# IBM/spark-s3-shuffle

Hardware: AMD Instinct MI355X
Metric: shuffle_block_compress_checksum_throughput (higher is better)
Workload: dtype u8; 1 GPU; terasort-10g-200p-lz4; direction=compress, codec=lz4, checksum=adler32, partitions_per_map_task=200, map_task_bytes=134217700, map_tasks_per_gpu=8, task_threads_per_gpu=4, map_tasks_per_library_call=2, inputs=resident in HBM

## Files before the change

### include/s3shuffle_codec.h

```cpp
#ifndef S3SHUFFLE_CODEC_H
#define S3SHUFFLE_CODEC_H

#include <stdint.h>

#ifdef __cplusplus
extern "C" {
#endif

#define S3S_ABI_VERSION 11

enum { S3S_CODEC_NONE = 0, S3S_CODEC_LZ4 = 1, S3S_CODEC_SNAPPY = 2,
       S3S_CODEC_LZF = 4,
       S3S_CODEC_ZSTD = 3  };
enum { S3S_CHECKSUM_NONE = 0, S3S_CHECKSUM_ADLER32 = 1, S3S_CHECKSUM_CRC32 = 2,
       S3S_CHECKSUM_CRC32C = 3  };

enum {
  S3S_OK = 0,
  S3S_E_INVALID = -1,
  S3S_E_CAPACITY = -2,
  S3S_E_BAD_FRAME = -3,
  S3S_E_CHECKSUM = -4,
  S3S_E_HIP = -5,
  S3S_E_UNSUPPORTED = -6,
  S3S_E_NOMEM = -7,
  S3S_STATUS_NOT_RUN = -100
};

enum {
  S3S_OPT_LZ4_BLOCK_SIZE = 1,
  S3S_OPT_SNAPPY_BLOCK_SIZE = 2,
  S3S_OPT_PROFILE = 3,
  S3S_OPT_LZ4_VARIANT = 4,
  S3S_OPT_LZ4_VARIANT_USED = 7,
  S3S_OPT_SNAPPY_VARIANT = 6,
  S3S_OPT_LZ4_DECODE_VARIANT = 5,
  S3S_OPT_LZ4_BLOCK_SIZE_LARGE = 8,
  S3S_OPT_ZSTD_COMPRESS = 9,
  S3S_OPT_LZF_COMPRESS = 10,
  S3S_OPT_IO_ENCRYPTION_KEY_BITS = 11
};

enum {
  S3S_STAGE_TOTAL = 0,
  S3S_STAGE_CODEC = 1,
  S3S_STAGE_ASSEMBLE = 2,
  S3S_STAGE_CHECKSUM = 3,
  S3S_STAGE_DISCOVER = 4,
  S3S_STAGE_HASH = 5,
  S3S_STAGE_COUNT = 6
};

typedef struct s3s_ctx s3s_ctx;

const char* s3s_version(void);
int s3s_abi_version(void);
int s3s_device_count(void);
s3s_ctx* s3s_create(int device_ordinal, int64_t scratch_bytes);
void s3s_destroy(s3s_ctx* ctx);
const char* s3s_last_error(const s3s_ctx* ctx);
int s3s_set_option(s3s_ctx* ctx, int key, int64_t value);
int64_t s3s_get_option(const s3s_ctx* ctx, int key);
int s3s_set_io_encryption(s3s_ctx* ctx, const uint8_t* key, int32_t key_bytes);
int s3s_set_stream_ivs(s3s_ctx* ctx, const uint8_t* ivs, int64_t n_ivs);
void* s3s_stream(const s3s_ctx* ctx);
double s3s_stage_ms(const s3s_ctx* ctx, int stage);

int64_t s3s_max_compressed_size(const s3s_ctx* ctx, int codec, const int64_t* src_offsets,
                                int32_t num_partitions);

int s3s_compress_map_output(s3s_ctx* ctx, int codec, int checksum_algo, const uint8_t* src,
                            const int64_t* src_offsets, int32_t num_partitions, uint8_t* dst,
                            int64_t dst_capacity, int64_t* out_index, int64_t* out_checksums,
// ... 105 lines not shown
```

### spark-s3-shuffle_amd/csrc/codec_api.hip

```cpp
#include "s3s_ctx.h"
#include <atomic>

using namespace s3s;

namespace {
inline void dbg_sync(s3s_ctx* ctx, const char* what) {
  static const bool on = getenv("S3S_DEBUG_SYNC") != nullptr;
  if (!on) return;
  const hipError_t e = hipStreamSynchronize(ctx->stream);
  fprintf(stderr, "[s3s] %s: %s\n", what, hipGetErrorString(e));
}
}

extern "C" {

const char* s3s_version(void) { return "s3shuffle-codec-mi355x 0.1.0 (gfx950)"; }
int s3s_abi_version(void) { return S3S_ABI_VERSION; }

int s3s_device_count(void) {
  int n = 0;
  if (hipGetDeviceCount(&n) != hipSuccess) return 0;
  return n;
}

s3s_ctx* s3s_create(int device_ordinal, int64_t scratch_bytes) {
  int n = 0;
  hipError_t e = hipGetDeviceCount(&n);
  if (e != hipSuccess || n <= 0) {
    fail(nullptr, S3S_E_HIP, "no HIP device available (%s); this library has no CPU fallback",
         e != hipSuccess ? hipGetErrorString(e) : "device count 0");
    return nullptr;
  }
  if (device_ordinal < 0 || device_ordinal >= n) {
    fail(nullptr, S3S_E_INVALID, "device ordinal %d out of range [0,%d)", device_ordinal, n);
    return nullptr;
  }
  s3s_ctx* ctx = new s3s_ctx();
  ctx->device = device_ordinal;
  auto bail = [&](const char* what, hipError_t err) -> s3s_ctx* {
    fail(nullptr, S3S_E_HIP, "%s failed: %s", what, hipGetErrorString(err));
    delete ctx;
    return nullptr;
  };
  if ((e = hipSetDevice(device_ordinal)) != hipSuccess) return bail("hipSetDevice", e);
  {
    int cus = 0;
    if (hipDeviceGetAttribute(&cus, hipDeviceAttributeMultiprocessorCount, device_ordinal) == hipSuccess && cus > 0) ctx->cu_count = cus;
  }
  if ((e = hipStreamCreateWithFlags(&ctx->stream, hipStreamNonBlocking)) != hipSuccess)
    return bail("hipStreamCreate", e);
  for (auto& ev : ctx->ev)
    if ((e = hipEventCreate(&ev)) != hipSuccess) return bail("hipEventCreate", e);
  if ((e = hipEventCreate(&ctx->ev_hash)) != hipSuccess) return bail("hipEventCreate", e);
  for (auto& ev : ctx->ev_auto)
    if ((e = hipEventCreate(&ev)) != hipSuccess) return bail("hipEventCreate", e);
  const size_t tb = checksum_tables_bytes();
  std::vector<uint8_t> host_tabs(tb);
  checksum_tables_build(host_tabs.data());
  if (ensure(ctx, B_TABLES, tb) != S3S_OK ||
      hipMemcpy(ctx->buf[B_TABLES].p, host_tabs.data(), tb, hipMemcpyHostToDevice) != hipSuccess) {
    fail(nullptr, S3S_E_HIP, "table upload failed: %s", ctx->err);
    s3s_destroy(ctx);
    return nullptr;
  }
  if (scratch_bytes > 0) (void)ensure(ctx, B_SLOTS, (size_t)scratch_bytes);
  return ctx;
}

void s3s_destroy(s3s_ctx* ctx) {
  if (!ctx) return;
  hipSetDevice(ctx->device);
  if (ctx->stream) hipStreamSynchronize(ctx->stream);
  if (ctx->hb_shared) {
    for (int i = 0; i < 2; i++) {
      if (ctx->hb_ev_in[i]) hipEventSynchronize(ctx->hb_ev_in[i]);
      if (ctx->hb_ev_out[i]) hipEventSynchronize(ctx->hb_ev_out[i]);
    }
  } else {
    if (ctx->hb_in) hipStreamSynchronize(ctx->hb_in);
    if (ctx->hb_out) hipStreamSynchronize(ctx->hb_out);
  }
  for (auto& b : ctx->buf)
    if (b.p) hipFree(b.p);
  if (ctx->h_stage) hipHostFree(ctx->h_stage);
  for (auto& ev : ctx->ev)
    if (ev) hipEventDestroy(ev);
  if (ctx->ev_hash) hipEventDestroy(ctx->ev_hash);
  for (auto& ev : ctx->ev_auto)
    if (ev) hipEventDestroy(ev);
  for (auto& ev : ctx->ev_up)
    if (ev) hipEventDestroy(ev);
  if (ctx->copy_stream) hipStreamDestroy(ctx->copy_stream);
  for (int i = 0; i < 2; i++) {
    if (ctx->hb_ev_in[i]) hipEventDestroy(ctx->hb_ev_in[i]);
    if (ctx->hb_ev_out[i]) hipEventDestroy(ctx->hb_ev_out[i]);
  }
  if (ctx->hb_in && !ctx->hb_shared) hipStreamDestroy(ctx->hb_in);
  if (ctx->hb_out && !ctx->hb_shared) hipStreamDestroy(ctx->hb_out);
  if (ctx->stream) hipStreamDestroy(ctx->stream);
  wipe(&ctx->enc_keys, sizeof ctx->enc_keys);
  delete ctx;
}

void* s3s_host_alloc(int64_t bytes) {
  if (bytes <= 0) return nullptr;
  void* p = nullptr;
  if (hipHostMalloc(&p, (size_t)bytes, hipHostMallocPortable) != hipSuccess) return nullptr;
  return p;
}

void s3s_host_free(void* p) {
  if (p) (void)hipHostFree(p);
}

const char* s3s_last_error(const s3s_ctx* ctx) { return ctx ? ctx->err : g_create_error; }

int s3s_set_option(s3s_ctx* ctx, int key, int64_t value) {
  if (!ctx) return S3S_E_INVALID;
  switch (key) {
    case S3S_OPT_LZ4_BLOCK_SIZE:
      if (value < 64) return fail(ctx, S3S_E_INVALID, "lz4 blockSize must be >= 64, got %lld", (long long)value);
      if (value > kLz4MaxBlock)
        return fail(ctx, S3S_E_UNSUPPORTED, "lz4 blockSize %lld > %d not supported", (long long)value, kLz4MaxBlock);
      ctx->lz4_block = value;
      return S3S_OK;
    case S3S_OPT_LZ4_BLOCK_SIZE_LARGE:
      if (value < 64) return fail(ctx, S3S_E_INVALID, "lz4 blockSize must be >= 64, got %lld", (long long)value);
      if (value > kBatchMaxBlock)
        return fail(ctx, S3S_E_UNSUPPORTED, "lz4 blockSize %lld > %d not supported", (long long)value, kBatchMaxBlock);
      ctx->lz4_block = value;
      return S3S_OK;
    case S3S_OPT_SNAPPY_BLOCK_SIZE:
      if (value <= 0) return fail(ctx, S3S_E_INVALID, "snappy blockSize must be > 0");
      if (value > kBatchMaxBlock)
        return fail(ctx, S3S_E_UNSUPPORTED, "snappy blockSize %lld > %d not supported", (long long)value, kBatchMaxBlock);
      ctx->snappy_block = value;
      return S3S_OK;
    case S3S_OPT_PROFILE:
      ctx->profile = value != 0;
      return S3S_OK;
    case S3S_OPT_ZSTD_COMPRESS:
      if (value != 0 && value != 1) return fail(ctx, S3S_E_INVALID, "zstd compress must be 0 or 1");
      ctx->zstd_compress = (int)value;
      return S3S_OK;
    case S3S_OPT_LZF_COMPRESS:
      if (value != 0 && value != 1) return fail(ctx, S3S_E_INVALID, "lzf compress must be 0 or 1");
      ctx->lzf_compress = (int)value;
      return S3S_OK;
    case S3S_OPT_LZ4_DECODE_VARIANT:
      if (value != 3 && value != 4) return fail(ctx, S3S_E_INVALID, "decode variant must be 3 (ring decoder) or 4 (batch decoder)");
      ctx->lz4_decode_variant = (int)value;
      return S3S_OK;
    case S3S_OPT_SNAPPY_VARIANT:
      if (value < 0 || value > 1) return fail(ctx, S3S_E_INVALID, "snappy variant must be 0..1");
      ctx->snappy_variant = (int)value;
      return S3S_OK;
    case S3S_OPT_LZ4_VARIANT:
      if (value != 1 && value != 9 && value != 10) return fail(ctx, S3S_E_INVALID, "lz4 variant must be 1 (general batch), 10 (exact windows) or 9 (auto)");
      ctx->lz4_variant = (int)value;
      ctx->auto_samples[0] = ctx->auto_samples[1] = 0;
      ctx->auto_tick = 0;
      return S3S_OK;
    case S3S_OPT_IO_ENCRYPTION_KEY_BITS:
      return fail(ctx, S3S_E_INVALID, "option %d is read-only (s3s_set_io_encryption switches the layer)", key);
  }
  return fail(ctx, S3S_E_INVALID, "unknown option %d", key);
}

int64_t s3s_get_option(const s3s_ctx* ctx, int key) {
  if (!ctx) return S3S_E_INVALID;
  switch (key) {
    case S3S_OPT_LZ4_BLOCK_SIZE:
    case S3S_OPT_LZ4_BLOCK_SIZE_LARGE: return ctx->lz4_block;
    case S3S_OPT_SNAPPY_BLOCK_SIZE: return ctx->snappy_block;
    case S3S_OPT_PROFILE: return ctx->profile;
    case S3S_OPT_LZ4_VARIANT: return ctx->lz4_variant;
    case S3S_OPT_LZ4_VARIANT_USED: return ctx->lz4_variant_used;
    case S3S_OPT_LZ4_DECODE_VARIANT: return ctx->lz4_decode_variant;
    case S3S_OPT_SNAPPY_VARIANT: return ctx->snappy_variant;
    case S3S_OPT_ZSTD_COMPRESS: return ctx->zstd_compress;
    case S3S_OPT_LZF_COMPRESS: return ctx->lzf_compress;
    case S3S_OPT_IO_ENCRYPTION_KEY_BITS: return ctx->enc_key_bits;
  }
  return S3S_E_INVALID;
}

int s3s_set_io_encryption(s3s_ctx* ctx, const uint8_t* key, int32_t key_bytes) {
  if (!ctx) return S3S_E_INVALID;
  ctx->err[0] = 0;
  if (!key || key_bytes == 0) {
    wipe(&ctx->enc_keys, sizeof ctx->enc_keys);
    ctx->enc_rounds = ctx->enc_key_bits = 0;
    ctx->enc_epoch++;
    return S3S_OK;
  }
  if (key_bytes != 16 && key_bytes != 24 && key_bytes != 32)
    return fail(ctx, S3S_E_INVALID, "IO encryption key must be 16, 24 or 32 bytes, got %d", (int)key_bytes);
  AesKeys fresh = {};
  const int rounds = aes_expand_key(key, key_bytes, &fresh);
  ctx->enc_keys = fresh;
  wipe(&fresh, sizeof fresh);
  ctx->enc_rounds = rounds;
  ctx->enc_key_bits = 8 * key_bytes;
  ctx->enc_epoch++;
  return S3S_OK;
}

int s3s_set_stream_ivs(s3s_ctx* ctx, const uint8_t* ivs, int64_t n_ivs) {
  if (!ctx) return S3S_E_INVALID;
  ctx->err[0] = 0;
  ctx->ivs.clear();
  ctx->ivs_set = false;
  if (n_ivs < 0 || (n_ivs > 0 && !ivs)) return fail(ctx, S3S_E_INVALID, "null IV array or negative count");
  if (n_ivs > 0x7fffffffll) return fail(ctx, S3S_E_INVALID, "more IVs than a call has partitions");
  ctx->ivs.assign(ivs, ivs + 16 * (size_t)n_ivs);
// ... 392 lines not shown
      k.status = s3s_compress_map_output_device(ctx, codec, checksum_algo, k.d_src, k.src_offsets, k.num_partitions,
                                                k.d_dst, k.dst_capacity, k.out_index, k.out_checksums, &k.out_total);
      if (k.status != S3S_OK && worst == S3S_OK) worst = k.status;
    }
    return verdict.finish(worst);
  }
  HIP_TRY(ctx, hipSetDevice(ctx->device));
  const int64_t bs = effective_block(ctx, codec);
  const int level = codec == S3S_CODEC_LZ4 ? lz4_level(bs) : 0;
  int64_t n_items64 = 0, n_chunks64 = 0, n_parts64 = 0;
  for (int32_t t = 0; t < n_tasks; t++) {
    const s3s_map_task& k = tasks[t];
    if (k.num_partitions < 0 || !k.src_offsets || !k.out_index || k.dst_capacity < 0)
      return fail(ctx, S3S_E_INVALID, "task %d: null offsets/index, negative partition count or capacity", t);
    if (checksum_algo != S3S_CHECKSUM_NONE && !k.out_checksums)
      return fail(ctx, S3S_E_INVALID, "task %d: out_checksums is null but a checksum algorithm is selected", t);
    for (int32_t p = 0; p < k.num_partitions; p++) {
      const int64_t u = k.src_offsets[p + 1] - k.src_offsets[p];
      if (u < 0) return fail(ctx, S3S_E_INVALID, "task %d: offsets not monotonic at %d", t, p);
      if (u > 0 && codec == S3S_CODEC_SNAPPY) {
        snappy_segment_counts(bs, u, &n_items64, &n_chunks64);
      } else if (u > 0) {
        const int64_t ch = (u + bs - 1) / bs;
        n_chunks64 += ch;
        n_items64 += ch + (codec != S3S_CODEC_LZF);
      }
    }
    const int64_t tu = k.num_partitions > 0 ? k.src_offsets[k.num_partitions] - k.src_offsets[0] : 0;
    if ((tu > 0 && !k.d_src) || (!k.d_dst && k.dst_capacity > 0)) return fail(ctx, S3S_E_INVALID, "task %d: null data pointer", t);
    n_parts64 += k.num_partitions;
  }
  if (n_items64 > 0x7fffff00ll) return fail(ctx, S3S_E_UNSUPPORTED, "too many codec blocks in one call");
  const int32_t n_items = (int32_t)n_items64, n_chunks = (int32_t)n_chunks64;
  const size_t np1 = (size_t)n_parts64 + (size_t)n_tasks;
  const size_t items_bytes = sizeof(Item) * (size_t)n_items;
  auto al = [](size_t x) { return (x + 15) & ~size_t(15); };
  const size_t o_items = 0, o_pf = al(o_items + items_bytes), o_seg = al(o_pf + 4 * np1), o_idx = al(o_seg + 4 * np1),
               o_sums = al(o_idx + 8 * np1), o_status = al(o_sums + 8 * ((size_t)n_parts64 + 1)),
               o_tails = al(o_status + 4 * (size_t)n_tasks + 16), stage_total = o_tails + sizeof(TaskTail) * (size_t)n_tasks + 16;
  int rc;
  if ((rc = ensure_stage(ctx, stage_total))) return rc;
  uint8_t* hs = static_cast<uint8_t*>(ctx->h_stage);
  Item* h_items = reinterpret_cast<Item*>(hs + o_items);
  int32_t* h_pf = reinterpret_cast<int32_t*>(hs + o_pf);
  int32_t* h_seg = reinterpret_cast<int32_t*>(hs + o_seg);
  int64_t* h_idx = reinterpret_cast<int64_t*>(hs + o_idx);
  int64_t* h_sums = reinterpret_cast<int64_t*>(hs + o_sums);
  int32_t* h_status = reinterpret_cast<int32_t*>(hs + o_status);
  TaskTail* h_tails = reinterpret_cast<TaskTail*>(hs + o_tails);
  std::vector<int32_t> first_item((size_t)n_tasks + 1), first_part((size_t)n_tasks + 1), first_seg((size_t)n_tasks + 1);
  const uint8_t* base = tasks[0].d_src;
  {
    int32_t it = 0, ch = 0, pp = 0, seg = 0;
    for (int32_t t = 0; t < n_tasks; t++) {
      const s3s_map_task& k = tasks[t];
      first_item[(size_t)t] = it;
      first_part[(size_t)t] = pp;
      first_seg[(size_t)t] = seg;
      const int64_t delta = k.d_src ? (int64_t)(k.d_src - base) : 0;
      int32_t* pf = h_pf + pp + t;
      int32_t* sg = h_seg + pp + t;
      int32_t seg_t = 0;
      for (int32_t p = 0; p < k.num_partitions; p++) {
        pf[p] = it - first_item[(size_t)t];
        sg[p] = seg_t;
        const int64_t u = k.src_offsets[p + 1] - k.src_offsets[p];
        seg_t += worst_segs(max_partition_size(codec, bs, u));
        if (u <= 0) continue;
        if (codec == S3S_CODEC_SNAPPY) h_items[it++] = Item{0, 0, kItemSnappyHeader, -1, p};
        if (codec == S3S_CODEC_ZSTD) h_items[it++] = Item{u, 0, kItemZstdHeader, -1, p};
        for (int64_t pos = 0; pos < u; pos += bs) {
          const int32_t len = (int32_t)((u - pos) < bs ? (u - pos) : bs);
          if (codec == S3S_CODEC_SNAPPY) {
            snappy_plan_chunk(h_items, it, ch, delta + k.src_offsets[p] + pos, len, p);
            continue;
          }
          if (codec == S3S_CODEC_ZSTD) {
            h_items[it++] = Item{delta + k.src_offsets[p] + pos, len, kItemZstdBlock | ((pos + len == u) << 8), ch++, p};
            continue;
          }
          if (codec == S3S_CODEC_LZF) {
            h_items[it++] = Item{delta + k.src_offsets[p] + pos, len, kItemLzfChunk, ch++, p};
            continue;
          }
          h_items[it++] = Item{delta + k.src_offsets[p] + pos, len, lz4_chunk_kind(len) | (level << 8), ch++, p};
        }
        if (codec == S3S_CODEC_LZ4) h_items[it++] = Item{0, 0, kItemLz4End | (level << 8), -1, p};
      }
      pf[k.num_partitions] = it - first_item[(size_t)t];
      sg[k.num_partitions] = seg_t;
      seg += seg_t;
      pp += k.num_partitions;
    }
    first_item[(size_t)n_tasks] = it;
    first_part[(size_t)n_tasks] = pp;
    first_seg[(size_t)n_tasks] = seg;
  }
  const int32_t total_segs = first_seg[(size_t)n_tasks];
  const int64_t slot_stride = codec == S3S_CODEC_SNAPPY ? snappy_slot_stride(bs) : codec_slot_stride(codec, bs);
  if ((rc = ensure(ctx, B_ITEMS, items_bytes + 16))) return rc;
  if ((rc = ensure(ctx, B_PART_FIRST, 4 * np1))) return rc;
  if ((rc = ensure(ctx, B_SEG_START, 4 * np1))) return rc;
  if ((rc = ensure(ctx, B_INDEX, 8 * np1))) return rc;
  if ((rc = ensure(ctx, B_SUMS, 8 * ((size_t)n_parts64 + 1)))) return rc;
  if ((rc = ensure(ctx, B_STATUS, 4 * (size_t)n_tasks + 16))) return rc;
  if ((rc = ensure(ctx, B_PARTIAL, 16 * (size_t)(total_segs > 0 ? total_segs : 1)))) return rc;
  if ((rc = ensure(ctx, B_SLOTS, (size_t)slot_stride * (size_t)(n_chunks > 0 ? n_chunks : 1)))) return rc;
  if ((rc = ensure(ctx, B_ITEM_SIZE, sizeof(uint32_t) * (size_t)(n_items + 1)))) return rc;
  if ((rc = ensure(ctx, B_ITEM_OFF, sizeof(int64_t) * ((size_t)n_items + (size_t)n_tasks + 1)))) return rc;
  if ((rc = ensure(ctx, B_ITEM_CHECK, sizeof(uint32_t) * (size_t)(n_items + 1)))) return rc;
  if ((rc = ensure(ctx, B_WORK, 64))) return rc;
  if ((rc = ensure(ctx, B_TAILS, sizeof(TaskTail) * (size_t)n_tasks + 16))) return rc;
  const int32_t zstd_grid = zstd_resident_groups(ctx, n_items);
  if (codec == S3S_CODEC_ZSTD && (rc = ensure(ctx, B_ZENC, (size_t)zstd_grid * (size_t)zstd_compress_scratch_stride()))) return rc;
  for (int32_t t = 0; t < n_tasks; t++) {
    const s3s_map_task& k = tasks[t];
    TaskTail& d = h_tails[t];
    d.first_item = first_item[(size_t)t];
    d.n_items = first_item[(size_t)t + 1] - first_item[(size_t)t];
    d.first_pp = first_part[(size_t)t] + t;
    d.n_parts = k.num_partitions;
    d.first_part = first_part[(size_t)t];
    d.first_seg = first_seg[(size_t)t];
    d.n_segs = first_seg[(size_t)t + 1] - first_seg[(size_t)t];
    d.pad = 0;
    d.data = k.d_dst;
    d.data_len = k.dst_capacity;
    d.dst = k.d_dst;
    d.dst_capacity = k.dst_capacity;
  }
  HIP_TRY(ctx, hipMemsetAsync(ctx->buf[B_STATUS].p, 0, 4 * (size_t)n_tasks + 16, ctx->stream));
  HIP_TRY(ctx, hipMemcpyAsync(ctx->buf[B_TAILS].p, h_tails, sizeof(TaskTail) * (size_t)n_tasks, hipMemcpyHostToDevice, ctx->stream));
  if (n_items > 0)
    HIP_TRY(ctx, hipMemcpyAsync(ctx->buf[B_ITEMS].p, h_items, items_bytes, hipMemcpyHostToDevice, ctx->stream));
  HIP_TRY(ctx, hipMemcpyAsync(ctx->buf[B_PART_FIRST].p, h_pf, 4 * np1, hipMemcpyHostToDevice, ctx->stream));
  HIP_TRY(ctx, hipMemcpyAsync(ctx->buf[B_SEG_START].p, h_seg, 4 * np1, hipMemcpyHostToDevice, ctx->stream));
  record(ctx, 0);
  if (codec == S3S_CODEC_LZ4) {
    const int variant = ctx->lz4_variant == 9 ? 10 : ctx->lz4_variant;
    ctx->lz4_variant_used = variant;
    launch_lz4_compress(base, dev<Item>(ctx, B_ITEMS), n_items, dev<uint32_t>(ctx, B_ITEM_CHECK),
                        dev<uint8_t>(ctx, B_SLOTS), (int32_t)slot_stride, dev<uint32_t>(ctx, B_ITEM_SIZE), dev<uint32_t>(ctx, B_WORK), lz4_resident_waves(ctx),
                        variant, ctx->stream,
                        ctx->profile ? ctx->ev_hash : nullptr, bs >= kLz4U32From);
  } else if (codec == S3S_CODEC_ZSTD) {
    launch_zstd_compress(base, dev<Item>(ctx, B_ITEMS), n_items, dev<uint8_t>(ctx, B_SLOTS), slot_stride, dev<uint32_t>(ctx, B_ITEM_SIZE),
                         dev<uint8_t>(ctx, B_ZENC), zstd_grid, ctx->stream);
  } else if (codec == S3S_CODEC_LZF) {
    launch_lzf_compress(base, dev<Item>(ctx, B_ITEMS), n_items, dev<uint8_t>(ctx, B_SLOTS), slot_stride, dev<uint32_t>(ctx, B_ITEM_SIZE),
                        ctx->stream);
  } else {
    launch_snappy_compress(base, dev<Item>(ctx, B_ITEMS), n_items, dev<uint8_t>(ctx, B_SLOTS), slot_stride,
                           dev<uint32_t>(ctx, B_ITEM_SIZE), ctx->snappy_variant, ctx->stream);
  }
  HIP_TRY(ctx, hipGetLastError());
  dbg_sync(ctx, "batch codec");
  record(ctx, 1);
  launch_scan_items_batch(dev<TaskTail>(ctx, B_TAILS), n_tasks, dev<uint32_t>(ctx, B_ITEM_SIZE), dev<int64_t>(ctx, B_ITEM_OFF),
                          dev<int32_t>(ctx, B_PART_FIRST), dev<int64_t>(ctx, B_INDEX), ctx->stream);
  dbg_sync(ctx, "batch scan");
  launch_gather_items_batch(dev<TaskTail>(ctx, B_TAILS), n_tasks, n_items, base, dev<Item>(ctx, B_ITEMS), dev<uint8_t>(ctx, B_SLOTS),
                            slot_stride, dev<uint32_t>(ctx, B_ITEM_SIZE), dev<int64_t>(ctx, B_ITEM_OFF), dev<int32_t>(ctx, B_STATUS),
                            ctx->stream);
  dbg_sync(ctx, "batch gather");
  HIP_TRY(ctx, hipGetLastError());
  record(ctx, 2);
  if (checksum_algo != S3S_CHECKSUM_NONE) {
    launch_checksum_batch(checksum_algo, dev<TaskTail>(ctx, B_TAILS), n_tasks, total_segs, (int32_t)n_parts64, dev<int64_t>(ctx, B_INDEX),
                          dev<int32_t>(ctx, B_SEG_START), ctx->buf[B_TABLES].p, dev<uint32_t>(ctx, B_PARTIAL), dev<int64_t>(ctx, B_SUMS),
                          ctx->stream);
    HIP_TRY(ctx, hipGetLastError());
  }
  record(ctx, 3);
  HIP_TRY(ctx, hipMemcpyAsync(h_idx, ctx->buf[B_INDEX].p, 8 * np1, hipMemcpyDeviceToHost, ctx->stream));
  if (checksum_algo != S3S_CHECKSUM_NONE && n_parts64 > 0)
    HIP_TRY(ctx, hipMemcpyAsync(h_sums, ctx->buf[B_SUMS].p, 8 * (size_t)n_parts64, hipMemcpyDeviceToHost, ctx->stream));
  HIP_TRY(ctx, hipMemcpyAsync(h_status, ctx->buf[B_STATUS].p, 4 * (size_t)n_tasks, hipMemcpyDeviceToHost, ctx->stream));
  HIP_TRY(ctx, hipStreamSynchronize(ctx->stream));
  if (ctx->profile) {
    float ms = 0;
    hipEventElapsedTime(&ms, ctx->ev[0], ctx->ev[3]); ctx->stage_ms[S3S_STAGE_TOTAL] = ms;
    hipEventElapsedTime(&ms, ctx->ev[0], ctx->ev[1]); ctx->stage_ms[S3S_STAGE_CODEC] = ms;
    ctx->stage_ms[S3S_STAGE_HASH] = 0;
    if (codec == S3S_CODEC_LZ4) {
      hipEventElapsedTime(&ms, ctx->ev[0], ctx->ev_hash); ctx->stage_ms[S3S_STAGE_HASH] = ms;
      hipEventElapsedTime(&ms, ctx->ev_hash, ctx->ev[1]); ctx->stage_ms[S3S_STAGE_CODEC] = ms;
    }
    hipEventElapsedTime(&ms, ctx->ev[1], ctx->ev[2]); ctx->stage_ms[S3S_STAGE_ASSEMBLE] = ms;
    hipEventElapsedTime(&ms, ctx->ev[2], ctx->ev[3]); ctx->stage_ms[S3S_STAGE_CHECKSUM] = ms;
    ctx->stage_ms[S3S_STAGE_DISCOVER] = 0;
  }
  int worst = S3S_OK;
  for (int32_t t = 0; t < n_tasks; t++) {
    s3s_map_task& k = tasks[t];
    const int32_t pp = first_part[(size_t)t] + t;
    memcpy(k.out_index, h_idx + pp, sizeof(int64_t) * ((size_t)k.num_partitions + 1));
    k.out_total = h_idx[pp + k.num_partitions];
    k.status = S3S_OK;
    if (h_status[t] != 0 || k.out_total > k.dst_capacity) {
      k.status = S3S_E_CAPACITY;
      if (worst == S3S_OK)
        worst = fail(ctx, S3S_E_CAPACITY, "task %d: dst_capacity %lld too small for %lld output bytes", t,
                     (long long)k.dst_capacity, (long long)k.out_total);
      continue;
    }
    if (checksum_algo != S3S_CHECKSUM_NONE && k.num_partitions > 0)
      memcpy(k.out_checksums, h_sums + first_part[(size_t)t], sizeof(int64_t) * (size_t)k.num_partitions);
  }
  return verdict.finish(worst);
}
// ... 205 lines not shown
```

### spark-s3-shuffle_amd/csrc/lz4_compress.hip

```cpp
#include "s3s_internal.h"
#include "lz4_window_engine.inc"

#ifdef S3S_LZ4_TIMING
__device__ unsigned long long g_lz4_dbg[32];
#define DBG_T(var) const unsigned long long var = __builtin_amdgcn_s_memtime()
#define DBG_ADD(slot, val) dbg[slot] += (val)
#else
#define DBG_T(var)
#define DBG_ADD(slot, val)
#endif

namespace s3s {
namespace {

constexpr int kMfLimit = 12, kLastLiterals = 5, kMinMatch = 4;

__device__ __forceinline__ uint32_t hash13(uint32_t v) { return (v * 2654435761u) >> 19; }

__device__ __forceinline__ uint32_t hash5_12(uint32_t v, uint32_t b4) {
  constexpr uint32_t kLo = 0x1BBCDCBBu, kHi = 0xCFu;
  const uint32_t p_lo = v * kLo;
  const uint32_t p_hi = __umulhi(v, kLo) + v * kHi + b4 * kLo;
  return ((p_lo >> 28) | (p_hi << 4)) & 0xfffu;
}
// ... 842 lines not shown
    }
#pragma unroll
    for (int gq = 0; gq < kDepth / 16; gq++) {
      uint32_t a = acc;
#pragma unroll
      for (int j = 0; j < 16; j++) a = rotl32(a + w[16 * gq + j] * XXP2, 13) * XXP1;
      acc = i + 16 * gq < s16 ? a : acc;
    }
    i = s16;
  }
  for (; i < stripes; i++) acc = rotl32(acc + ld(16 * i + 4 * k) * XXP2, 13) * XXP1;
  const int q0 = lane & ~3;
  const uint32_t v1 = (uint32_t)__shfl((int)acc, q0), v2 = (uint32_t)__shfl((int)acc, q0 + 1),
                 v3 = (uint32_t)__shfl((int)acc, q0 + 2), v4 = (uint32_t)__shfl((int)acc, q0 + 3);
  uint32_t h = len >= 16 ? rotl32(v1, 1) + rotl32(v2, 7) + rotl32(v3, 12) + rotl32(v4, 18) : seed + XXP5;
  h += (uint32_t)len;
  if (mine && k == 0) {
    int p = stripes << 4;
    for (; p + 4 <= len; p += 4) h = rotl32(h + ld(p) * XXP3, 17) * XXP4;
    for (; p < len; p++) h = rotl32(h + (uint32_t)g[p] * XXP5, 11) * XXP1;
    h ^= h >> 15;
    h *= XXP2;
    h ^= h >> 13;
    h *= XXP3;
    h ^= h >> 16;
    item_check[it] = h;
  }
}

}

void launch_lz4_compress(const uint8_t* d_src, const Item* d_items, int32_t n_items,
                         uint32_t* d_item_check, uint8_t* d_slots, int32_t slot_stride, uint32_t* d_item_size, uint32_t* d_work, int resident_waves,
                         int variant, hipStream_t st, hipEvent_t after_hash, bool has_u32) {
  if (n_items <= 0) {
    if (after_hash) hipEventRecord(after_hash, st);
    return;
  }
  static const int xxh_env = getenv("S3S_XXH") ? atoi(getenv("S3S_XXH")) : -1;
  const int xxh_mode = xxh_env >= 0 ? xxh_env : 2;
  if (xxh_mode == 0)
    hipLaunchKernelGGL(xxh32_items_wave_kernel<kItemLz4Chunk>, dim3((unsigned)n_items), dim3(kWave), 0, st, d_src, d_items,
                       n_items, kLz4BlockSeed, d_item_check);
  else if (xxh_mode == 2)
    hipLaunchKernelGGL(xxh32_items_quad_kernel<false>, dim3((unsigned)((n_items + 15) / 16)), dim3(kWave), 0, st, d_src, d_items,
                       n_items, kLz4BlockSeed, d_item_check);
  else
    hipLaunchKernelGGL(xxh32_items_quad_kernel<true>, dim3((unsigned)((n_items + 15) / 16)), dim3(kWave), 0, st, d_src, d_items,
                       n_items, kLz4BlockSeed, d_item_check);
  if (has_u32)
    hipLaunchKernelGGL(xxh32_items_wave_kernel<kItemLz4ChunkU32>, dim3((unsigned)n_items), dim3(kWave), 0, st, d_src, d_items,
                       n_items, kLz4BlockSeed, d_item_check);
  if (after_hash) hipEventRecord(after_hash, st);
  (void)hipMemsetAsync(d_work, 0, sizeof(uint32_t), st);
  static const int grid_env = getenv("S3S_LZ4_GRID") ? atoi(getenv("S3S_LZ4_GRID")) : 0;
  int grid = grid_env > 0 ? grid_env : resident_waves;
  if (grid > n_items) grid = n_items;
  if (variant == 1)
    hipLaunchKernelGGL(lz4_compress_l2_kernel<false>, dim3((unsigned)grid), dim3(kWave), 0, st, d_src,
                       d_items, n_items, slot_stride, d_item_check, d_slots, d_item_size, d_work);
  else
    hipLaunchKernelGGL(lz4_compress_l2_kernel<true>, dim3((unsigned)grid), dim3(kWave), 0, st, d_src,
                       d_items, n_items, slot_stride, d_item_check, d_slots, d_item_size, d_work);
  if (has_u32)
    hipLaunchKernelGGL(lz4_compress_u32_kernel, dim3((unsigned)n_items), dim3(kWave), 0, st, d_src, d_items, n_items,
                       slot_stride, d_item_check, d_slots, d_item_size);
}

}
```

### spark-s3-shuffle_amd/csrc/s3s_ctx.h

```cpp
#pragma once
#include <stdarg.h>
#include <stdio.h>
#include <stdlib.h>
#include <string.h>

#include <vector>

#include "s3s_internal.h"

namespace s3s {

inline thread_local char g_create_error[512] = "";

struct DevBuf {
  void* p = nullptr;
  size_t cap = 0;
};

enum BufId {
  B_ITEMS, B_PART_FIRST, B_SLOTS, B_ITEM_SIZE, B_ITEM_OFF, B_INDEX, B_SUMS, B_SEG_START,
  B_PARTIAL, B_STATUS, B_TABLES, B_SRC, B_DST, B_OFFSETS, B_FRAMES, B_PART_NFRAMES,
  B_FRAME_OUT, B_REF_SUMS, B_ITEM_CHECK, B_RANGES, B_TILE_RANGE,
  B_HB_IN0, B_HB_IN1, B_HB_OUT0, B_HB_OUT1,
  B_WORK,
  B_PARTIAL2,
  B_ZSCRATCH, B_ZPIECES,
  B_ZENC,
  B_TAILS,
  B_IVS,
  B_CRYPT,
  B_CRYPT_OFF,
  B_COUNT
};

}

struct s3s_ctx {
  int device = 0;
  hipStream_t stream = nullptr;
  char err[512] = "";
  int64_t lz4_block = 32768;
  int64_t snappy_block = 32768;
  int profile = 0;
  int lz4_variant = 10;
  int auto_choice = 1;
  int auto_samples[2] = {0, 0};
  int auto_tick = 0;
  double auto_ms_per_mib[2] = {0, 0};
  int lz4_variant_used = 0;
  hipEvent_t ev_auto[2] = {nullptr, nullptr};
  int lz4_decode_variant = 4;
  int snappy_variant = 1;
  int zstd_compress = 0;
  int lzf_compress = 0;
  s3s::DevBuf buf[s3s::B_COUNT];
  int cu_count = 256;
  void* h_stage = nullptr;
  size_t h_stage_cap = 0;
  hipEvent_t ev[S3S_STAGE_COUNT + 1] = {};
  hipEvent_t ev_hash = nullptr;
  hipStream_t copy_stream = nullptr;
  std::vector<hipEvent_t> ev_up;
  const uint8_t* up_host = nullptr;
  hipStream_t hb_in = nullptr, hb_out = nullptr;
  bool hb_shared = false;
  hipEvent_t hb_ev_in[2] = {nullptr, nullptr}, hb_ev_out[2] = {nullptr, nullptr};
  double stage_ms[S3S_STAGE_COUNT] = {};
  s3s::AesKeys enc_keys = {};
  int enc_rounds = 0, enc_key_bits = 0;
  uint64_t enc_epoch = 0;
  bool enc_suspended = false;
  std::vector<uint8_t> ivs;
// ... 215 lines not shown
```

### spark-s3-shuffle_amd/csrc/s3s_internal.h

```cpp
#pragma once
#include <hip/hip_runtime.h>
#include <stdint.h>

#include "../../include/s3shuffle_codec.h"

namespace s3s {

constexpr int kWave = 64;
constexpr int kMaxBlock = 32768;
constexpr int kLz4MaxBlock = 65536;
constexpr int kLz4U32From = 65536 + 11;
constexpr int kBatchMaxBlock = 1 << 25;
constexpr int kSnappyFragment = 65536;
constexpr int kSlotHeader = 32;
constexpr int kLz4FrameHeader = 21;
constexpr int kSnappyStreamHeader = 16;
constexpr uint32_t kLz4BlockSeed = 0x9747b28cu;

enum : int32_t {
  kItemLz4Chunk = 0,
  kItemLz4End = 1,
  kItemSnappyHeader = 2,
  kItemSnappyChunk = 3,
  kItemSnappyChunkHead = 4,
  kItemSnappyFrag = 5,
  kItemLz4ChunkU32 = 6,
  kItemZstdHeader = 7,
  kItemZstdBlock = 8,
  kItemLzfChunk = 9,
  kItemIv = 10
};
constexpr int kLzfChunk = 65535;
constexpr int kLzfSlotPayload = (kLzfChunk + kLzfChunk / 32 + 4 + 15) & ~15;
constexpr int kZstdBlock = 1 << 17;
constexpr int kZstdFrameHeader = 14;

__host__ __device__ constexpr int snappy_varint_len(int64_t n) {
  return n < (1 << 7) ? 1 : n < (1 << 14) ? 2 : n < (1 << 21) ? 3 : n < (1 << 28) ? 4 : 5;
}

struct Item {
  int64_t src_off;
  int32_t len;
  int32_t kind;
  int32_t chunk;
  int32_t part;
};

constexpr uint32_t kRawFlag = 0x80000000u;

void launch_lz4_compress(const uint8_t* d_src, const Item* d_items, int32_t n_items,
                         uint32_t* d_item_check, uint8_t* d_slots, int32_t slot_stride, uint32_t* d_item_size, uint32_t* d_work, int resident_waves,
                         int variant, hipStream_t st, hipEvent_t after_hash = nullptr, bool has_u32 = false);
bool snappy_compress_available();
void launch_snappy_compress(const uint8_t* d_src, const Item* d_items, int32_t n_items,
                            uint8_t* d_slots, int64_t slot_stride, uint32_t* d_item_size,
                            int variant, hipStream_t st);
int64_t zstd_compress_scratch_stride();
void launch_zstd_compress(const uint8_t* d_src, const Item* d_items, int32_t n_items, uint8_t* d_slots, int64_t slot_stride,
                          uint32_t* d_item_size, uint8_t* d_scratch, int32_t grid, hipStream_t st);
void launch_lzf_compress(const uint8_t* d_src, const Item* d_items, int32_t n_items, uint8_t* d_slots, int64_t slot_stride,
                         uint32_t* d_item_size, hipStream_t st);
struct AesKeys {
  uint32_t rk[60];
};
int aes_expand_key(const uint8_t* key, int key_bytes, AesKeys* keys);
enum { kCtrInPlace = 0, kCtrFromPlain = 1, kCtrDecrypt = 2 };
int64_t aes_ctr_max_bytes();
void launch_aes_ctr(int mode, const AesKeys& keys, int rounds, const uint8_t* d_in, uint8_t* d_out, const int64_t* d_stored_off,
                    const int64_t* d_plain_off, const uint8_t* d_ivs, int32_t n_parts, int64_t stored_bound, int64_t stored_limit,
                    hipStream_t st);
struct AesWindowIv {
  uint32_t w[4];
};
void launch_aes_ctr_window(const AesKeys& keys, int rounds, const AesWindowIv& iv0, const uint8_t* d_in, uint8_t* d_out,
                           const int64_t* d_stored_off, const int64_t* d_plain_off, uint8_t* d_iv_out, int32_t n_pieces, int64_t front,
                           int64_t window_len, hipStream_t st);
void launch_seed_iv_items(const Item* d_items, int32_t n_items, uint32_t* d_item_size, hipStream_t st);
void launch_scan_items(const Item* d_items, const uint32_t* d_item_size, int32_t n_items,
                       int64_t* d_item_off, const int32_t* d_part_first, int32_t n_parts,
                       int64_t* d_index, hipStream_t st);
void launch_gather_items(const uint8_t* d_src, const Item* d_items, int32_t n_items,
                         const uint8_t* d_slots, int64_t slot_stride, const uint32_t* d_item_size,
                         const int64_t* d_item_off, uint8_t* d_dst, int64_t dst_capacity,
                         int32_t* d_status, hipStream_t st);
size_t checksum_tables_bytes();
// ... 120 lines not shown
```

### spark-s3-shuffle_amd/s3shuffle/codec.py

```python
from __future__ import annotations

import ctypes
import os
from typing import Optional, Sequence, Tuple

import numpy as np

CODEC_NONE, CODEC_LZ4, CODEC_SNAPPY = 0, 1, 2
CODEC_ZSTD = 3
CODEC_LZF = 4
CHECKSUM_NONE, CHECKSUM_ADLER32, CHECKSUM_CRC32, CHECKSUM_CRC32C = 0, 1, 2, 3

OPT_LZ4_BLOCK_SIZE, OPT_SNAPPY_BLOCK_SIZE, OPT_PROFILE = 1, 2, 3
STAGE_TOTAL, STAGE_CODEC, STAGE_ASSEMBLE, STAGE_CHECKSUM, STAGE_DISCOVER, STAGE_HASH = 0, 1, 2, 3, 4, 5
OPT_LZ4_VARIANT = 4
OPT_LZ4_DECODE_VARIANT = 5
OPT_SNAPPY_VARIANT = 6
OPT_LZ4_VARIANT_USED = 7
OPT_LZ4_BLOCK_SIZE_LARGE = 8

OPT_ZSTD_COMPRESS = 9
OPT_LZF_COMPRESS = 10
OPT_IO_ENCRYPTION_KEY_BITS = 11

E_INVALID, E_CAPACITY, E_BAD_FRAME, E_CHECKSUM, E_HIP, E_UNSUPPORTED, E_NOMEM = -1, -2, -3, -4, -5, -6, -7
STATUS_NOT_RUN = -100
_ERR_NAMES = {
    E_INVALID: "S3S_E_INVALID",
    E_CAPACITY: "S3S_E_CAPACITY",
    E_BAD_FRAME: "S3S_E_BAD_FRAME",
    E_CHECKSUM: "S3S_E_CHECKSUM",
    E_HIP: "S3S_E_HIP",
    E_UNSUPPORTED: "S3S_E_UNSUPPORTED",
    E_NOMEM: "S3S_E_NOMEM",
}

_PKG_ROOT = os.path.dirname(os.path.dirname(os.path.abspath(__file__)))


class CodecError(RuntimeError):

    def __init__(self, code: int, message: str, partition: int = -1):
        super().__init__(f"{_ERR_NAMES.get(code, code)}: {message}")
        self.code = code
        self.partition = partition


def library_path() -> str:
    override = os.environ.get("S3S_CODEC_LIB")
    if override:
        return override
    return os.path.join(_PKG_ROOT, "lib", "libs3shuffle_codec.so")


class MapTask(ctypes.Structure):
# ... 476 lines not shown
```

Before: 98.08 GB/s.

## Pack batch plan into one upload/download buffer and assign per-context stream priority classes

Host-side staging for the batch compress path is packed into a single contiguous plan buffer. One host-to-device copy replaces several memsets and copies, and one device-to-host copy replaces three readbacks. The LZ4 work counter is zeroed on the host and uploaded with the plan, so its separate memset is dropped. Each context's stream is also given a priority class (lowest, normal or highest) based on its creation slot and the hardware queue cap, with the aim of spreading concurrent task threads across hardware queues. The priority assignment could also create unfairness between contexts.

```diff
diff --git a/include/s3shuffle_codec.h b/include/s3shuffle_codec.h
--- a/include/s3shuffle_codec.h
+++ b/include/s3shuffle_codec.h
@@ -38,7 +38,8 @@
   S3S_OPT_LZ4_BLOCK_SIZE_LARGE = 8,
   S3S_OPT_ZSTD_COMPRESS = 9,
   S3S_OPT_LZF_COMPRESS = 10,
-  S3S_OPT_IO_ENCRYPTION_KEY_BITS = 11
+  S3S_OPT_IO_ENCRYPTION_KEY_BITS = 11,
+  S3S_OPT_STREAM_CLASS = 12
 };
 
 enum {
diff --git a/spark-s3-shuffle_amd/csrc/codec_api.hip b/spark-s3-shuffle_amd/csrc/codec_api.hip
--- a/spark-s3-shuffle_amd/csrc/codec_api.hip
+++ b/spark-s3-shuffle_amd/csrc/codec_api.hip
@@ -1,5 +1,6 @@
 #include "s3s_ctx.h"
 #include <atomic>
+#include <mutex>
 
 using namespace s3s;
 
@@ -9,6 +10,47 @@
   if (!on) return;
   const hipError_t e = hipStreamSynchronize(ctx->stream);
   fprintf(stderr, "[s3s] %s: %s\n", what, hipGetErrorString(e));
+}
+
+struct StreamSlots {
+  std::mutex mu;
+  uint64_t used = 0;
+};
+StreamSlots g_stream_slots[64];
+
+int hw_queue_cap() {
+  const char* e = getenv("GPU_MAX_HW_QUEUES");
+  const int cap = e ? atoi(e) : 4;
+  return cap < 1 ? 1 : (cap > 32 ? 32 : cap);
+}
+
+hipError_t create_placed_stream(s3s_ctx* ctx) {
+  static const int order = getenv("S3S_STREAM_POOLS") ? atoi(getenv("S3S_STREAM_POOLS")) : 1;
+  int least = 0, greatest = 0;
+  if (order != 0 && hipDeviceGetStreamPriorityRange(&least, &greatest) != hipSuccess) least = greatest = 0;
+  const int levels = least - greatest + 1;
+  StreamSlots& S = g_stream_slots[ctx->device & 63];
+  {
+    std::lock_guard<std::mutex> g(S.mu);
+    for (int i = 0; i < 64; i++)
+      if (!(S.used >> i & 1)) {
+        S.used |= uint64_t(1) << i;
+        ctx->stream_slot = i;
+        break;
+      }
+  }
+  ctx->stream_class = stream_class_ordered(ctx->stream_slot >= 0 ? ctx->stream_slot : 64, hw_queue_cap(), levels, order);
+  if (ctx->stream_class == kStreamLowest) return hipStreamCreateWithPriority(&ctx->stream, hipStreamNonBlocking, least);
+  if (ctx->stream_class == kStreamHighest) return hipStreamCreateWithPriority(&ctx->stream, hipStreamNonBlocking, greatest);
+  return hipStreamCreateWithFlags(&ctx->stream, hipStreamNonBlocking);
+}
+
+void release_stream_slot(s3s_ctx* ctx) {
+  if (ctx->stream_slot < 0) return;
+  StreamSlots& S = g_stream_slots[ctx->device & 63];
+  std::lock_guard<std::mutex> g(S.mu);
+  S.used &= ~(uint64_t(1) << ctx->stream_slot);
+  ctx->stream_slot = -1;
 }
 }
 
@@ -39,6 +81,7 @@
   ctx->device = device_ordinal;
   auto bail = [&](const char* what, hipError_t err) -> s3s_ctx* {
     fail(nullptr, S3S_E_HIP, "%s failed: %s", what, hipGetErrorString(err));
+    release_stream_slot(ctx);
     delete ctx;
     return nullptr;
   };
@@ -47,8 +90,7 @@
     int cus = 0;
     if (hipDeviceGetAttribute(&cus, hipDeviceAttributeMultiprocessorCount, device_ordinal) == hipSuccess && cus > 0) ctx->cu_count = cus;
   }
-  if ((e = hipStreamCreateWithFlags(&ctx->stream, hipStreamNonBlocking)) != hipSuccess)
-    return bail("hipStreamCreate", e);
+  if ((e = create_placed_stream(ctx)) != hipSuccess) return bail("hipStreamCreate", e);
   for (auto& ev : ctx->ev)
     if ((e = hipEventCreate(&ev)) != hipSuccess) return bail("hipEventCreate", e);
   if ((e = hipEventCreate(&ctx->ev_hash)) != hipSuccess) return bail("hipEventCreate", e);
@@ -98,6 +140,7 @@
   if (ctx->hb_in && !ctx->hb_shared) hipStreamDestroy(ctx->hb_in);
   if (ctx->hb_out && !ctx->hb_shared) hipStreamDestroy(ctx->hb_out);
   if (ctx->stream) hipStreamDestroy(ctx->stream);
+  release_stream_slot(ctx);
   wipe(&ctx->enc_keys, sizeof ctx->enc_keys);
   delete ctx;
 }
@@ -163,6 +206,8 @@
       return S3S_OK;
     case S3S_OPT_IO_ENCRYPTION_KEY_BITS:
       return fail(ctx, S3S_E_INVALID, "option %d is read-only (s3s_set_io_encryption switches the layer)", key);
+    case S3S_OPT_STREAM_CLASS:
+      return fail(ctx, S3S_E_INVALID, "option %d is read-only (the context's creation slot decides it)", key);
   }
   return fail(ctx, S3S_E_INVALID, "unknown option %d", key);
 }
@@ -181,6 +226,7 @@
     case S3S_OPT_ZSTD_COMPRESS: return ctx->zstd_compress;
     case S3S_OPT_LZF_COMPRESS: return ctx->lzf_compress;
     case S3S_OPT_IO_ENCRYPTION_KEY_BITS: return ctx->enc_key_bits;
+    case S3S_OPT_STREAM_CLASS: return ctx->stream_class;
   }
   return S3S_E_INVALID;
 }
@@ -639,22 +685,19 @@
   }
   if (n_items64 > 0x7fffff00ll) return fail(ctx, S3S_E_UNSUPPORTED, "too many codec blocks in one call");
   const int32_t n_items = (int32_t)n_items64, n_chunks = (int32_t)n_chunks64;
-  const size_t np1 = (size_t)n_parts64 + (size_t)n_tasks;
-  const size_t items_bytes = sizeof(Item) * (size_t)n_items;
-  auto al = [](size_t x) { return (x + 15) & ~size_t(15); };
-  const size_t o_items = 0, o_pf = al(o_items + items_bytes), o_seg = al(o_pf + 4 * np1), o_idx = al(o_seg + 4 * np1),
-               o_sums = al(o_idx + 8 * np1), o_status = al(o_sums + 8 * ((size_t)n_parts64 + 1)),
-               o_tails = al(o_status + 4 * (size_t)n_tasks + 16), stage_total = o_tails + sizeof(TaskTail) * (size_t)n_tasks + 16;
+  const PackedPlan L = packed_plan((size_t)n_tasks, (size_t)n_parts64, (size_t)n_items, sizeof(TaskTail), sizeof(Item));
   int rc;
-  if ((rc = ensure_stage(ctx, stage_total))) return rc;
+  if ((rc = ensure_stage(ctx, L.total))) return rc;
   uint8_t* hs = static_cast<uint8_t*>(ctx->h_stage);
-  Item* h_items = reinterpret_cast<Item*>(hs + o_items);
-  int32_t* h_pf = reinterpret_cast<int32_t*>(hs + o_pf);
-  int32_t* h_seg = reinterpret_cast<int32_t*>(hs + o_seg);
-  int64_t* h_idx = reinterpret_cast<int64_t*>(hs + o_idx);
-  int64_t* h_sums = reinterpret_cast<int64_t*>(hs + o_sums);
-  int32_t* h_status = reinterpret_cast<int32_t*>(hs + o_status);
-  TaskTail* h_tails = reinterpret_cast<TaskTail*>(hs + o_tails);
+  Item* h_items = reinterpret_cast<Item*>(hs + L.items);
+  int32_t* h_pf = reinterpret_cast<int32_t*>(hs + L.part_first);
+  int32_t* h_seg = reinterpret_cast<int32_t*>(hs + L.seg_start);
+  int64_t* h_idx = reinterpret_cast<int64_t*>(hs + L.index);
+  int64_t* h_sums = reinterpret_cast<int64_t*>(hs + L.sums);
+  int32_t* h_status = reinterpret_cast<int32_t*>(hs + L.status);
+  TaskTail* h_tails = reinterpret_cast<TaskTail*>(hs + L.tails);
+  memset(hs + L.work, 0, 16);
+  memset(h_status, 0, L.up_end - L.status);
   std::vector<int32_t> first_item((size_t)n_tasks + 1), first_part((size_t)n_tasks + 1), first_seg((size_t)n_tasks + 1);
   const uint8_t* base = tasks[0].d_src;
   {
@@ -705,19 +748,20 @@
   }
   const int32_t total_segs = first_seg[(size_t)n_tasks];
   const int64_t slot_stride = codec == S3S_CODEC_SNAPPY ? snappy_slot_stride(bs) : codec_slot_stride(codec, bs);
-  if ((rc = ensure(ctx, B_ITEMS, items_bytes + 16))) return rc;
-  if ((rc = ensure(ctx, B_PART_FIRST, 4 * np1))) return rc;
-  if ((rc = ensure(ctx, B_SEG_START, 4 * np1))) return rc;
-  if ((rc = ensure(ctx, B_INDEX, 8 * np1))) return rc;
-  if ((rc = ensure(ctx, B_SUMS, 8 * ((size_t)n_parts64 + 1)))) return rc;
-  if ((rc = ensure(ctx, B_STATUS, 4 * (size_t)n_tasks + 16))) return rc;
+  if ((rc = ensure(ctx, B_PLAN, L.total))) return rc;
   if ((rc = ensure(ctx, B_PARTIAL, 16 * (size_t)(total_segs > 0 ? total_segs : 1)))) return rc;
   if ((rc = ensure(ctx, B_SLOTS, (size_t)slot_stride * (size_t)(n_chunks > 0 ? n_chunks : 1)))) return rc;
   if ((rc = ensure(ctx, B_ITEM_SIZE, sizeof(uint32_t) * (size_t)(n_items + 1)))) return rc;
   if ((rc = ensure(ctx, B_ITEM_OFF, sizeof(int64_t) * ((size_t)n_items + (size_t)n_tasks + 1)))) return rc;
   if ((rc = ensure(ctx, B_ITEM_CHECK, sizeof(uint32_t) * (size_t)(n_items + 1)))) return rc;
-  if ((rc = ensure(ctx, B_WORK, 64))) return rc;
-  if ((rc = ensure(ctx, B_TAILS, sizeof(TaskTail) * (size_t)n_tasks + 16))) return rc;
+  uint8_t* d_plan = dev<uint8_t>(ctx, B_PLAN);
+  const Item* d_items = reinterpret_cast<const Item*>(d_plan + L.items);
+  const TaskTail* d_tails = reinterpret_cast<const TaskTail*>(d_plan + L.tails);
+  const int32_t* d_pf = reinterpret_cast<const int32_t*>(d_plan + L.part_first);
+  const int32_t* d_seg = reinterpret_cast<const int32_t*>(d_plan + L.seg_start);
+  int32_t* d_status = reinterpret_cast<int32_t*>(d_plan + L.status);
+  int64_t* d_index = reinterpret_cast<int64_t*>(d_plan + L.index);
+  int64_t* d_sums = reinterpret_cast<int64_t*>(d_plan + L.sums);
   const int32_t zstd_grid = zstd_resident_groups(ctx, n_items);
   if (codec == S3S_CODEC_ZSTD && (rc = ensure(ctx, B_ZENC, (size_t)zstd_grid * (size_t)zstd_compress_scratch_stride()))) return rc;
   for (int32_t t = 0; t < n_tasks; t++) {
@@ -736,53 +780,46 @@
     d.dst = k.d_dst;
     d.dst_capacity = k.dst_capacity;
   }
-  HIP_TRY(ctx, hipMemsetAsync(ctx->buf[B_STATUS].p, 0, 4 * (size_t)n_tasks + 16, ctx->stream));
-  HIP_TRY(ctx, hipMemcpyAsync(ctx->buf[B_TAILS].p, h_tails, sizeof(TaskTail) * (size_t)n_tasks, hipMemcpyHostToDevice, ctx->stream));
-  if (n_items > 0)
-    HIP_TRY(ctx, hipMemcpyAsync(ctx->buf[B_ITEMS].p, h_items, items_bytes, hipMemcpyHostToDevice, ctx->stream));
-  HIP_TRY(ctx, hipMemcpyAsync(ctx->buf[B_PART_FIRST].p, h_pf, 4 * np1, hipMemcpyHostToDevice, ctx->stream));
-  HIP_TRY(ctx, hipMemcpyAsync(ctx->buf[B_SEG_START].p, h_seg, 4 * np1, hipMemcpyHostToDevice, ctx->stream));
+  HIP_TRY(ctx, hipMemcpyAsync(d_plan, hs, L.up_end, hipMemcpyHostToDevice, ctx->stream));
   record(ctx, 0);
   if (codec == S3S_CODEC_LZ4) {
     const int variant = ctx->lz4_variant == 9 ? 10 : ctx->lz4_variant;
     ctx->lz4_variant_used = variant;
-    launch_lz4_compress(base, dev<Item>(ctx, B_ITEMS), n_items, dev<uint32_t>(ctx, B_ITEM_CHECK),
-                        dev<uint8_t>(ctx, B_SLOTS), (int32_t)slot_stride, dev<uint32_t>(ctx, B_ITEM_SIZE), dev<uint32_t>(ctx, B_WORK), lz4_resident_waves(ctx),
+    launch_lz4_compress(base, d_items, n_items, dev<uint32_t>(ctx, B_ITEM_CHECK),
+                        dev<uint8_t>(ctx, B_SLOTS), (int32_t)slot_stride, dev<uint32_t>(ctx, B_ITEM_SIZE), reinterpret_cast<uint32_t*>(d_plan + L.work), lz4_resident_waves(ctx),
                         variant, ctx->stream,
-                        ctx->profile ? ctx->ev_hash : nullptr, bs >= kLz4U32From);
+                        ctx->profile ? ctx->ev_hash : nullptr, bs >= kLz4U32From, true);
   } else if (codec == S3S_CODEC_ZSTD) {
-    launch_zstd_compress(base, dev<Item>(ctx, B_ITEMS), n_items, dev<uint8_t>(ctx, B_SLOTS), slot_stride, dev<uint32_t>(ctx, B_ITEM_SIZE),
+    launch_zstd_compress(base, d_items, n_items, dev<uint8_t>(ctx, B_SLOTS), slot_stride, dev<uint32_t>(ctx, B_ITEM_SIZE),
                          dev<uint8_t>(ctx, B_ZENC), zstd_grid, ctx->stream);
   } else if (codec == S3S_CODEC_LZF) {
-    launch_lzf_compress(base, dev<Item>(ctx, B_ITEMS), n_items, dev<uint8_t>(ctx, B_SLOTS), slot_stride, dev<uint32_t>(ctx, B_ITEM_SIZE),
+    launch_lzf_compress(base, d_items, n_items, dev<uint8_t>(ctx, B_SLOTS), slot_stride, dev<uint32_t>(ctx, B_ITEM_SIZE),
                         ctx->stream);
   } else {
-    launch_snappy_compress(base, dev<Item>(ctx, B_ITEMS), n_items, dev<uint8_t>(ctx, B_SLOTS), slot_stride,
+    launch_snappy_compress(base, d_items, n_items, dev<uint8_t>(ctx, B_SLOTS), slot_stride,
                            dev<uint32_t>(ctx, B_ITEM_SIZE), ctx->snappy_variant, ctx->stream);
   }
   HIP_TRY(ctx, hipGetLastError());
   dbg_sync(ctx, "batch codec");
   record(ctx, 1);
-  launch_scan_items_batch(dev<TaskTail>(ctx, B_TAILS), n_tasks, dev<uint32_t>(ctx, B_ITEM_SIZE), dev<int64_t>(ctx, B_ITEM_OFF),
-                          dev<int32_t>(ctx, B_PART_FIRST), dev<int64_t>(ctx, B_INDEX), ctx->stream);
+  launch_scan_items_batch(d_tails, n_tasks, dev<uint32_t>(ctx, B_ITEM_SIZE), dev<int64_t>(ctx, B_ITEM_OFF),
+                          d_pf, d_index, ctx->stream);
   dbg_sync(ctx, "batch scan");
-  launch_gather_items_batch(dev<TaskTail>(ctx, B_TAILS), n_tasks, n_items, base, dev<Item>(ctx, B_ITEMS), dev<uint8_t>(ctx, B_SLOTS),
-                            slot_stride, dev<uint32_t>(ctx, B_ITEM_SIZE), dev<int64_t>(ctx, B_ITEM_OFF), dev<int32_t>(ctx, B_STATUS),
+  launch_gather_items_batch(d_tails, n_tasks, n_items, base, d_items, dev<uint8_t>(ctx, B_SLOTS),
+                            slot_stride, dev<uint32_t>(ctx, B_ITEM_SIZE), dev<int64_t>(ctx, B_ITEM_OFF), d_status,
                             ctx->stream);
   dbg_sync(ctx, "batch gather");
   HIP_TRY(ctx, hipGetLastError());
   record(ctx, 2);
   if (checksum_algo != S3S_CHECKSUM_NONE) {
-    launch_checksum_batch(checksum_algo, dev<TaskTail>(ctx, B_TAILS), n_tasks, total_segs, (int32_t)n_parts64, dev<int64_t>(ctx, B_INDEX),
-                          dev<int32_t>(ctx, B_SEG_START), ctx->buf[B_TABLES].p, dev<uint32_t>(ctx, B_PARTIAL), dev<int64_t>(ctx, B_SUMS),
+    launch_checksum_batch(checksum_algo, d_tails, n_tasks, total_segs, (int32_t)n_parts64, d_index,
+                          d_seg, ctx->buf[B_TABLES].p, dev<uint32_t>(ctx, B_PARTIAL), d_sums,
                           ctx->stream);
     HIP_TRY(ctx, hipGetLastError());
   }
   record(ctx, 3);
-  HIP_TRY(ctx, hipMemcpyAsync(h_idx, ctx->buf[B_INDEX].p, 8 * np1, hipMemcpyDeviceToHost, ctx->stream));
-  if (checksum_algo != S3S_CHECKSUM_NONE && n_parts64 > 0)
-    HIP_TRY(ctx, hipMemcpyAsync(h_sums, ctx->buf[B_SUMS].p, 8 * (size_t)n_parts64, hipMemcpyDeviceToHost, ctx->stream));
-  HIP_TRY(ctx, hipMemcpyAsync(h_status, ctx->buf[B_STATUS].p, 4 * (size_t)n_tasks, hipMemcpyDeviceToHost, ctx->stream));
+  HIP_TRY(ctx, hipMemcpyAsync(h_status, d_status, (checksum_algo != S3S_CHECKSUM_NONE ? L.total : L.sums) - L.status, hipMemcpyDeviceToHost,
+                              ctx->stream));
   HIP_TRY(ctx, hipStreamSynchronize(ctx->stream));
   if (ctx->profile) {
     float ms = 0;
diff --git a/spark-s3-shuffle_amd/csrc/lz4_compress.hip b/spark-s3-shuffle_amd/csrc/lz4_compress.hip
--- a/spark-s3-shuffle_amd/csrc/lz4_compress.hip
+++ b/spark-s3-shuffle_amd/csrc/lz4_compress.hip
@@ -898,7 +898,7 @@
 
 void launch_lz4_compress(const uint8_t* d_src, const Item* d_items, int32_t n_items,
                          uint32_t* d_item_check, uint8_t* d_slots, int32_t slot_stride, uint32_t* d_item_size, uint32_t* d_work, int resident_waves,
-                         int variant, hipStream_t st, hipEvent_t after_hash, bool has_u32) {
+                         int variant, hipStream_t st, hipEvent_t after_hash, bool has_u32, bool work_is_zero) {
   if (n_items <= 0) {
     if (after_hash) hipEventRecord(after_hash, st);
     return;
@@ -918,7 +918,7 @@
     hipLaunchKernelGGL(xxh32_items_wave_kernel<kItemLz4ChunkU32>, dim3((unsigned)n_items), dim3(kWave), 0, st, d_src, d_items,
                        n_items, kLz4BlockSeed, d_item_check);
   if (after_hash) hipEventRecord(after_hash, st);
-  (void)hipMemsetAsync(d_work, 0, sizeof(uint32_t), st);
+  if (!work_is_zero) (void)hipMemsetAsync(d_work, 0, sizeof(uint32_t), st);
   static const int grid_env = getenv("S3S_LZ4_GRID") ? atoi(getenv("S3S_LZ4_GRID")) : 0;
   int grid = grid_env > 0 ? grid_env : resident_waves;
   if (grid > n_items) grid = n_items;
diff --git a/spark-s3-shuffle_amd/csrc/s3s_ctx.h b/spark-s3-shuffle_amd/csrc/s3s_ctx.h
--- a/spark-s3-shuffle_amd/csrc/s3s_ctx.h
+++ b/spark-s3-shuffle_amd/csrc/s3s_ctx.h
@@ -7,6 +7,7 @@
 #include <vector>
 
 #include "s3s_internal.h"
+#include "stream_placement.h"
 
 namespace s3s {
 
@@ -30,6 +31,7 @@
   B_IVS,
   B_CRYPT,
   B_CRYPT_OFF,
+  B_PLAN,
   B_COUNT
 };
 
@@ -38,6 +40,8 @@
 struct s3s_ctx {
   int device = 0;
   hipStream_t stream = nullptr;
+  int stream_slot = -1;
+  int stream_class = 1;
   char err[512] = "";
   int64_t lz4_block = 32768;
   int64_t snappy_block = 32768;
diff --git a/spark-s3-shuffle_amd/csrc/s3s_internal.h b/spark-s3-shuffle_amd/csrc/s3s_internal.h
--- a/spark-s3-shuffle_amd/csrc/s3s_internal.h
+++ b/spark-s3-shuffle_amd/csrc/s3s_internal.h
@@ -51,7 +51,7 @@
 
 void launch_lz4_compress(const uint8_t* d_src, const Item* d_items, int32_t n_items,
                          uint32_t* d_item_check, uint8_t* d_slots, int32_t slot_stride, uint32_t* d_item_size, uint32_t* d_work, int resident_waves,
-                         int variant, hipStream_t st, hipEvent_t after_hash = nullptr, bool has_u32 = false);
+                         int variant, hipStream_t st, hipEvent_t after_hash = nullptr, bool has_u32 = false, bool work_is_zero = false);
 bool snappy_compress_available();
 void launch_snappy_compress(const uint8_t* d_src, const Item* d_items, int32_t n_items,
                             uint8_t* d_slots, int64_t slot_stride, uint32_t* d_item_size,
diff --git a/spark-s3-shuffle_amd/csrc/stream_placement.h b/spark-s3-shuffle_amd/csrc/stream_placement.h
--- /dev/null
+++ b/spark-s3-shuffle_amd/csrc/stream_placement.h
@@ -0,0 +1,57 @@
+#pragma once
+#include <stddef.h>
+#include <stdint.h>
+
+namespace s3s {
+
+enum StreamClass { kStreamLowest = 0, kStreamNormal = 1, kStreamHighest = 2, kStreamOverflow = 3 };
+
+inline int stream_pool_share(int cls, int cap, int levels) {
+  if (cap < 1) cap = 1;
+  if (cap > 32) cap = 32;
+  switch (cls) {
+    case kStreamLowest: return levels >= 3 ? cap : 0;
+    case kStreamNormal: return cap - 1;
+    case kStreamHighest: return levels >= 2 && cap > 2 ? cap - 2 : 0;
+  }
+  return 0;
+}
+
+inline int stream_class_ordered(int slot, int cap, int levels, int order) {
+  if (order == 0) return kStreamNormal;
+  static const int kOrders[2][3] = {{kStreamLowest, kStreamNormal, kStreamHighest}, {kStreamNormal, kStreamHighest, kStreamLowest}};
+  int first = 0;
+  for (int i = 0; i < 3; i++) {
+    const int cls = kOrders[order == 2 ? 1 : 0][i];
+    first += stream_pool_share(cls, cap, levels);
+    if (slot < first) return cls;
+  }
+  return kStreamOverflow;
+}
+
+inline int stream_class(int slot, int cap, int levels) { return stream_class_ordered(slot, cap, levels, 1); }
+
+struct PackedPlan {
+  size_t work, tails, items, part_first, seg_start, status, up_end;
+  size_t index, sums, total;
+};
+
+inline size_t plan_align(size_t x) { return (x + 15) & ~size_t(15); }
+
+inline PackedPlan packed_plan(size_t n_tasks, size_t n_parts, size_t n_items, size_t tail_bytes, size_t item_bytes) {
+  PackedPlan L;
+  const size_t np1 = n_parts + n_tasks;
+  L.work = 0;
+  L.tails = 16;
+  L.items = plan_align(L.tails + tail_bytes * n_tasks);
+  L.part_first = plan_align(L.items + item_bytes * n_items);
+  L.seg_start = plan_align(L.part_first + 4 * np1);
+  L.status = plan_align(L.seg_start + 4 * np1);
+  L.up_end = plan_align(L.status + 4 * n_tasks);
+  L.index = L.up_end;
+  L.sums = plan_align(L.index + 8 * np1);
+  L.total = plan_align(L.sums + 8 * n_parts);
+  return L;
+}
+
+}
diff --git a/spark-s3-shuffle_amd/s3shuffle/codec.py b/spark-s3-shuffle_amd/s3shuffle/codec.py
--- a/spark-s3-shuffle_amd/s3shuffle/codec.py
+++ b/spark-s3-shuffle_amd/s3shuffle/codec.py
@@ -21,6 +21,7 @@
 
 OPT_ZSTD_COMPRESS = 9
 OPT_LZF_COMPRESS = 10
+OPT_STREAM_CLASS = 12
 OPT_IO_ENCRYPTION_KEY_BITS = 11
 
 E_INVALID, E_CAPACITY, E_BAD_FRAME, E_CHECKSUM, E_HIP, E_UNSUPPORTED, E_NOMEM = -1, -2, -3, -4, -5, -6, -7
```

Result: faster. 115.1 GB/s, median of 6 (+17.4%).
